# BaratiLab/LNS-Latent-Neural-PDE-Solver

Hardware: AMD Instinct MI355X
Metric: rollout-steps/sec (encode+N latent steps+decode), NS2d 128^2 3-ch (higher is better)
Workload: dtype f32 (f16x2 split operands on the fp16 MFMA pipe, fp32 accumulate; fp32 tensors in HBM); 1 GPU; NS2d 128x128 3-channel, 64-step latent rollout, batch=64 per GPU (BASELINE.json configs[1]); preset=ns2d_128, batch_per_gpu=64, rollout_steps=64, global_batch=64, parallelism=trajectory-sharded x1, streams=propagator + 3 decode streams per GPU

## Files before the change

include/lns.h:

```cpp
#ifndef LNS_H_
#define LNS_H_

#include <stddef.h>
#include <stdint.h>

#ifdef __cplusplus
extern "C" {
#endif

#define LNS_ABI_VERSION 2
#define LNS_MAX_STAGES 8
#define LNS_MAX_KEY 160

#define LNS_OK 0
#define LNS_EINVAL (-1)
#define LNS_ENOKEY (-2)
#define LNS_ESTATE (-3)
#define LNS_ENOMEM (-4)
#define LNS_EHIP (-5)
#define LNS_ENONFINITE (-6)

#define LNS_AE_NONE 0
#define LNS_AE_SQUARE 1
#define LNS_AE_NONSQUARED 2
// ... 459 lines not shown
                          double* lam, int32_t* status, void* stream);
int lns_op_ensemble_transform(const float* z, const double* X, int B, int M, int64_t n, float* out, void* stream);

int lns_op_energy_spectrum(const float* yhat, const float* y , int B, int T, int C, int H, int W,
                           const lns_eval_spec* spec, float* out, void* stream);
int lns_op_energy_spectrum_basis(const float* yhat, const float* y , int B, int T, int C, int H, int W,
                                 const lns_eval_spec* spec, float* out, void* stream, int basis_y, int basis_x);

int lns_op_field_stats(const float* yhat, const float* y, int B, int T, int C, int H, int W, const lns_eval_spec* spec,
                       const lns_stats_spec* hspec , float* stats_out, int32_t* hist_out ,
                       void* stream);

int lns_op_flow_stats(const float* yhat, const float* y, int B, int T, int C, int H, int W, const lns_eval_spec* spec,
                      const lns_flow_spec* fspec, float* flow_out, int32_t* hist_out , void* stream);
int lns_op_vorticity(const float* fields, int B, int T, int C, int H, int W, const lns_eval_spec* spec,
                     const lns_flow_spec* fspec, float* vort_out, void* stream);

int lns_time_maps_state_bytes(int B, int C, int H, int W, size_t* bytes);
int lns_op_time_maps(const float* yhat, const float* y, int B, int T, int C, int H, int W, const lns_eval_spec* spec,
                     int map_from, int map_every, float* maps_out, void* state, size_t state_bytes, void* stream);

int lns_op_eval_attrib(const float* yhat, const float* r, const float* y, int B, int T, int C, int H, int W,
                       const lns_eval_spec* spec, float* prop_frame, float* prop_seq, float* cross_frame, float* cross_seq,
                       void* stream);

int lns_op_latent_err(const float* z, const float* ztrue, int B, int T, int zper, int64_t zstride, float eps, float* frame_out,
                      float* seq_out, void* stream);

int lns_op_groupnorm_stats(const float* x, int B, int C, int HW, int groups, float eps,
                           const float* gamma_host, const float* beta_host, const float* premul,
                           float* ss, void* stream);
int lns_op_attention(const float* qkv, int B, int heads, int dim_head, int n, float scale,
                     float* o, void* stream);
int lns_op_fa_sandwich(const float* u, const float* kx, const float* ky, int B, int heads, int C,
                       int H, int W, float eps, int apply_instance_norm, float* out, void* stream);
int lns_op_fa_pool(const float* x, int64_t x_bs, const float* ss, int B, int C, int H, int W,
                   float* mx, float* my, void* stream);

int lns_op_fourier_block(const float* x, int B, int Cin, int Cout, int H, int W, int m1, int m2, const float* w1_host,
                         const float* w2_host, const float* conv_w_host, const float* conv_b_host,
                         const float* cond, const float* freq_w_host, const float* freq_b_host,
                         const float* lin_w_host, const float* lin_b_host, int activation, int residual,
                         float* y, void* stream);

typedef struct lns_fourier_block lns_fourier_block;
int lns_fourier_block_create(int Cin, int Cout, int m1, int m2, const float* w1_host, const float* w2_host,
                             const float* conv_w_host, const float* conv_b_host, const float* freq_w_host,
                             const float* freq_b_host, const float* lin_w_host, const float* lin_b_host, int activation,
                             int residual, int device, lns_fourier_block** out);
int lns_fourier_block_forward(lns_fourier_block* h, const float* x, const float* cond, int B, int H, int W, float* y,
                              void* stream);
void lns_fourier_block_destroy(lns_fourier_block* h);

int lns_metric_rel_l2(const float* yhat, const float* y, int B, int T, int C, int HW, float mean, float std, float eps,
                      float* frame_out, float* seq_out, float* scratch, void* stream);

#define LNS_METRIC_ZERO_WALLS 1
#define LNS_METRIC_CLAMP 2
int lns_metric_rel_l2_ch(const float* yhat, const float* y, int B, int T, int C, int H, int W, const float* mean_host,
                         const float* std_host, const int* flags_host, float clamp_lo, float clamp_hi, float eps,
                         float* frame_out, float* seq_out, float* scratch, void* stream);

#ifdef __cplusplus
}
#endif
#endif
// ... 1 lines not shown
```

lns-latent-neural-pde-solver_amd/_lib.py:

```python
import ctypes
import os
import subprocess

_HERE = os.path.dirname(os.path.abspath(__file__))
LIB_PATH = os.environ.get("LNS_HIP_LIB") or os.path.join(_HERE, "liblns_hip.so")
CSRC = os.path.join(_HERE, "csrc")

LNS_MAX_STAGES = 8
LNS_ABI_VERSION = 2
LNS_AE_NONE, LNS_AE_SQUARE, LNS_AE_NONSQUARED, LNS_AE_HALF_PERIODIC = 0, 1, 2, 3
LNS_PROP_NONE, LNS_PROP_PLAIN, LNS_PROP_CONDITIONAL = 0, 1, 2
LNS_PAD_ZEROS, LNS_PAD_CIRCULAR = 0, 1
LNS_SPECTRUM_DFT, LNS_SPECTRUM_DCT = 0, 1
LNS_OK, LNS_EINVAL, LNS_ENOKEY, LNS_ESTATE, LNS_ENOMEM, LNS_EHIP, LNS_ENONFINITE = 0, -1, -2, -3, -4, -5, -6


class LnsLibraryError(RuntimeError):
    pass


class LnsError(RuntimeError):
    pass


# ... 159 lines not shown


SYMBOLS = [
    "lns_create_error", "lns_create", "lns_destroy", "lns_last_error", "lns_num_params",
    "lns_param_info", "lns_set_weight", "lns_finalize_weights", "lns_latent_shape", "lns_prepare",
    "lns_encode", "lns_encode_cond", "lns_encode_affine", "lns_decode", "lns_propagate", "lns_rollout", "lns_rollout_latent", "lns_check_finite", "lns_set_option",
    "lns_rollout_eval_workspace_bytes", "lns_rollout_eval", "lns_rollout_latent_eval",
    "lns_rollout_select_workspace_bytes", "lns_rollout_select", "lns_rollout_latent_select",
    "lns_rollout_ensemble_workspace_bytes", "lns_rollout_latent_ensemble", "lns_op_ensemble_stats",
    "lns_rollout_latent_ensemble_eval", "lns_op_ensemble_score",
    "lns_rollout_latent_ensemble_quantiles", "lns_op_ensemble_quantiles",
    "lns_rollout_latent_ensemble_exceed", "lns_op_ensemble_exceed",
    "lns_rollout_ensemble_analysis_workspace_bytes", "lns_rollout_latent_ensemble_analysis",
    "lns_op_ensemble_obs_gram", "lns_op_etkf_transform", "lns_op_ensemble_transform",
    "lns_spectrum_bins", "lns_rollout_eval_spectrum", "lns_rollout_latent_eval_spectrum", "lns_op_energy_spectrum",
    "lns_spectrum_bins_basis", "lns_op_energy_spectrum_basis",
    "lns_rollout_eval_stats", "lns_rollout_latent_eval_stats", "lns_op_field_stats",
    "lns_rollout_eval_maps_workspace_bytes", "lns_rollout_eval_maps", "lns_rollout_latent_eval_maps",
    "lns_time_maps_state_bytes", "lns_op_time_maps",
    "lns_rollout_eval_attrib_workspace_bytes", "lns_rollout_eval_attrib", "lns_rollout_latent_eval_attrib",
    "lns_autoencode_eval_workspace_bytes", "lns_autoencode_eval", "lns_op_eval_attrib", "lns_op_latent_err",
    "lns_rollout_eval_flow", "lns_rollout_latent_eval_flow", "lns_op_flow_stats", "lns_op_vorticity",
    "lns_train_workspace_bytes", "lns_train_forward", "lns_train_backward",
    "lns_loss_smooth_l1", "lns_adam_step", "lns_adam_step_tensors", "lns_train_step_workspace_bytes", "lns_train_step",
    "lns_grad_norm_scratch_bytes", "lns_grad_norm_tensors", "lns_grad_scale_tensors", "lns_update_step_tensors",
    "lns_train_step_clip_workspace_bytes", "lns_train_step_clip",
    "lns_train_backward_ex", "lns_loss_obs_mse_scratch_bytes", "lns_loss_obs_mse", "lns_fit_step_workspace_bytes", "lns_fit_step",
    "lns_train_tangent_workspace_bytes", "lns_train_tangent", "lns_op_orthonormalize",
    "lns_trace_enable", "lns_trace_count", "lns_trace_info", "lns_trace_copy",
    "lns_timing_enable", "lns_timing_count", "lns_timing_info", "lns_timing_mfma_flops", "lns_build_has",
    "lns_op_conv_wgrad_scratch_bytes", "lns_op_conv_wgrad",
    "lns_op_groupnorm_train", "lns_op_gelu_grad", "lns_op_bias_grad",
    "lns_op_fa_reducer", "lns_fa_reducer_fits", "lns_op_fa_lrk", "lns_fa_lrk_fits", "lns_rotary_table", "lns_op_ln_pe", "lns_op_apply",
    "lns_op_conv2d", "lns_op_conv_gn", "lns_op_fa_fused", "lns_op_conv_pair_stress", "lns_op_groupnorm_stats", "lns_op_attention", "lns_op_fa_sandwich", "lns_op_fa_pool", "lns_op_fourier_block",
    "lns_fourier_block_create", "lns_fourier_block_forward", "lns_fourier_block_destroy", "lns_metric_rel_l2", "lns_metric_rel_l2_ch",
]

_lib = None


def build(force=False):
    srcs = [os.path.join(CSRC, f) for f in os.listdir(CSRC)
            if f.endswith((".hip", ".cpp", ".h", ".inc"))] + [os.path.join(_HERE, "..", "include", "lns.h")]
    if (not force and os.path.exists(LIB_PATH)
            and all(os.path.getmtime(LIB_PATH) >= os.path.getmtime(s) for s in srcs)):
        return LIB_PATH
    subprocess.check_call(["make", "-s", "-j4", "-C", CSRC])
    return LIB_PATH


def lib():
    global _lib
    if _lib is not None:
        return _lib
    if not os.path.exists(LIB_PATH):
        raise LnsLibraryError(
            "HIP extension %s is missing; run `python -c 'import __graft_entry__ as g; g.build()'` "
            "(there is no CPU fallback for the LNS hot path)" % LIB_PATH)
    try:
        L = ctypes.CDLL(LIB_PATH)
    except OSError as e:
        raise LnsLibraryError("cannot load %s: %s" % (LIB_PATH, e))
    c = ctypes
    vp, i, i64p, fp = c.c_void_p, c.c_int, c.POINTER(c.c_int64), c.POINTER(c.c_float)
    if os.environ.get("LNS_HIP_LIB"):
        def _absent(*_a, **_k):
            raise LnsLibraryError("entry point missing from the library selected by LNS_HIP_LIB")
# ... 133 lines not shown
    L.lns_build_has.argtypes = [c.c_char_p]
    L.lns_trace_enable.argtypes = [vp, i]
    L.lns_trace_count.argtypes = [vp]
    L.lns_trace_info.argtypes = [vp, i, c.c_char_p, i, i64p]
    L.lns_trace_copy.argtypes = [vp, i, vp]
    L.lns_timing_enable.argtypes = [vp, i]
    L.lns_timing_count.argtypes = [vp]
    L.lns_timing_info.argtypes = [vp, i, c.c_char_p, i, c.POINTER(c.c_double), i64p,
                                  c.POINTER(c.c_double), c.POINTER(c.c_double)]
    L.lns_timing_mfma_flops.argtypes = [vp, i, c.POINTER(c.c_double)]
    L.lns_op_conv2d.argtypes = [vp, i, i, i, i, i, i, vp, vp, i, i, i, i, i, i, i, i, i, i,
                                vp, i, i, vp, vp, vp, i, vp, vp]
    if hasattr(L, "lns_op_conv_gn"):
        L.lns_op_conv_gn.argtypes = [c.POINTER(LnsConvGnArgs), vp]
    if hasattr(L, "lns_op_fa_fused"):
        L.lns_op_fa_fused.argtypes = [c.POINTER(LnsFaFusedArgs), vp]
    if hasattr(L, "lns_op_fa_reducer"):
        L.lns_op_fa_reducer.argtypes = [c.POINTER(LnsFaReducerArgs), vp]
        L.lns_fa_reducer_fits.argtypes = [i, i, i, i]
        L.lns_op_fa_lrk.argtypes = [c.POINTER(LnsFaLrkArgs), vp]
        L.lns_fa_lrk_fits.argtypes = [i, i]
        L.lns_rotary_table.argtypes = [i, vp, i, vp]
        L.lns_op_ln_pe.argtypes = [vp, c.c_int64, i, i, i, vp, vp, vp, i, c.c_float, vp, fp, vp]
        L.lns_op_apply.argtypes = [vp, c.c_int64, vp, i, i, i, i, vp, vp, vp]
    if hasattr(L, "lns_op_conv_wgrad"):
        L.lns_op_conv_wgrad_scratch_bytes.argtypes = [i, i, i, i, i, i, i, c.POINTER(c.c_size_t)]
        L.lns_op_conv_wgrad.argtypes = [vp, vp, i, i, i, i, i, i, i, i, i, i, i, vp, vp, c.c_size_t, vp]
    if hasattr(L, "lns_op_groupnorm_train"):
        L.lns_op_groupnorm_train.argtypes = [vp, i, i, i, i, c.c_float, vp, vp, vp, vp, vp, vp, vp, vp, vp, i, vp, vp]
        L.lns_op_gelu_grad.argtypes = [vp, vp, vp, c.c_int64, vp]
        L.lns_op_bias_grad.argtypes = [vp, i, i, i, vp, i, vp]
    L.lns_op_groupnorm_stats.argtypes = [vp, i, i, i, i, c.c_float, vp, vp, vp, vp, vp]
    L.lns_op_attention.argtypes = [vp, i, i, i, i, c.c_float, vp, vp]
    L.lns_op_fa_sandwich.argtypes = [vp, vp, vp, i, i, i, i, i, c.c_float, i, vp, vp]
    L.lns_op_fa_pool.argtypes = [vp, c.c_int64, vp, i, i, i, i, vp, vp, vp]
    L.lns_op_fourier_block.argtypes = [vp, i, i, i, i, i, i, i, vp, vp, vp, vp, vp, vp, vp, vp, vp, i, i, vp, vp]
    L.lns_fourier_block_create.argtypes = [i, i, i, i, vp, vp, vp, vp, vp, vp, vp, vp, i, i, i, c.POINTER(vp)]
    L.lns_fourier_block_forward.argtypes = [vp, vp, vp, i, i, i, vp, vp]
    L.lns_fourier_block_destroy.argtypes = [vp]
    L.lns_fourier_block_destroy.restype = None
    L.lns_metric_rel_l2.argtypes = [vp, vp, i, i, i, i, c.c_float, c.c_float, c.c_float, vp, vp, vp, vp]
    L.lns_metric_rel_l2.restype = i
    L.lns_metric_rel_l2_ch.argtypes = [vp, vp, i, i, i, i, i, vp, vp, vp, c.c_float, c.c_float, c.c_float, vp, vp, vp, vp]
    L.lns_metric_rel_l2_ch.restype = i
    _lib = L
    return L
```

lns-latent-neural-pde-solver_amd/csrc/lns_engine.cpp:

```cpp
#include <algorithm>
#include <cmath>
#include <cstdarg>
#include <cstdio>
#include <cstdlib>
#include <cstring>
#include <memory>
#include <mutex>
#include <tuple>
#include <stdexcept>

#include "lns_conv_launch.h"
#include "lns_engine.h"
#include "lns_fold.h"
#include "lns_op_scratch.h"
#include "lns_resolve.h"
#include "lns_spectrum.h"

#define LNS_MAX_BATCH 65535

namespace lns {
void build_model(lns_engine* e);

static thread_local std::string g_create_error;

// ... 480 lines not shown
        TRef out = conv_same3(h1, l.conv2, 1, l.mode_y, l.mode_x, ACT_NONE, &skip, 0, l.name + ".conv2", raw_out);
        free_t(h1);
        if (skip_owned) free_t(skip);
        return out;
    }

    TRef lower_sa(const Layer& l, TRef x, bool raw_out) {
        if (x.pending()) throw std::runtime_error("SABlock input must be materialised");
        const int n = x.H * x.W, inner = l.heads * l.dim_head;
        if (l.pe >= 0 && n > l.pe_len) throw std::runtime_error("SABlock: more tokens than positional table rows");
        TRef h = alloc_t(x.C, x.H, x.W);
        h.amax_const = ln_pe_bound(x.C, vec_absmax(l.ln_g), vec_absmax(l.ln_b), vec_absmax(l.pe));
        {
            Op op;
            op.type = OP_LNPE; op.name = l.name + ".ln_pe"; op.cls = CLS_LNPE;
            memset(&op.ln, 0, sizeof op.ln);
            op.ln.x = as_ptr<const float>(x.ptr); op.ln.x_bs = x.bs; op.ln.C = x.C; op.ln.n = n; op.ln.eps = 1e-5f;
            op.ln.gamma = as_ptr<const float>(vecp(l.ln_g)); op.ln.beta = as_ptr<const float>(vecp(l.ln_b));
            op.ln.pe_t = as_ptr<const float>(vecp(l.pe)); op.ln.pe_stride = l.pe_len;
            op.ln.h = as_ptr<float>(h.ptr); op.ln.B = B;
            op.bytes = 2.0 * B * x.C * n * 4;
            plan->ops.push_back(op);
        }
        TRef qkv = conv_same1(h, l.qkv, ACT_NONE, nullptr, nullptr, l.name + ".qkv");
        free_t(h);
        TRef o = alloc_t(inner, x.H, x.W);
        o.amax = qkv.amax;
        {
            Op op;
            op.type = OP_ATTN; op.name = l.name + ".attn"; op.cls = CLS_ATTN;
            op.at.qkv = as_ptr<const float>(qkv.ptr); op.at.B = B; op.at.heads = l.heads; op.at.D = l.dim_head;
            op.at.n = n; op.at.scale = (float)std::pow((double)l.dim_head, -0.5); op.at.o = as_ptr<float>(o.ptr);
            op.at.amax_in = qkv.amax ? as_ptr<const unsigned>(qkv.amax) : nullptr;
            op.flops = 4.0 * B * l.heads * (double)n * n * l.dim_head;
            {
                const bool f16 = op.at.amax_in != nullptr && getenv("LNS_ATTN_FP32") == nullptr;
                const double np_ = (n + 31) / 32 * 32;
                op.mfma_flops = 4.0 * B * l.heads * np_ * np_ * l.dim_head * (f16 ? 3.0 : 1.0);
                op.form = f16 ? "f16x2 attention" : "fp32 MFMA attention";
            }
            op.bytes = 4.0 * B * 4.0 * inner * n;
            plan->ops.push_back(op);
        }
        free_t(qkv);
        TRef out = conv_same1(o, l.proj, ACT_NONE, &x, nullptr, l.name + ".proj_out", -1, raw_out);
        free_t(o);
        return out;
    }

    uint64_t rotary_table(int n, const std::string& invf_key) {
        const Param& p = e->params[e->pindex.at(invf_key)];
        const int half = (int)p.numel();
        std::vector<float> cs((size_t)n * half * 2);
        rotary_table_fill(n, p.host.data(), half, cs.data());
        return const_floats(cs);
    }

    int next_chunk_group = 1;
    int fa_chunk_samples(size_t bytes_per_sample) const {
        const long cap = (long)e->opt_fa_chunk_mb << 20;
        if (cap <= 0 || (long)bytes_per_sample * B <= cap) return 0;
        const int chunk = (int)std::max<long>(1, cap / (long)bytes_per_sample);
        return chunk >= B ? 0 : chunk;
    }
    void chunk_fa_chain(size_t inproj_at, size_t sandwich_at, size_t toout_at, size_t bytes_per_sample) {
        const int chunk = fa_chunk_samples(bytes_per_sample);
// ... 1036 lines not shown

using namespace lns;

struct DeviceGuard {
    int prev = -1; bool switched = false;
    explicit DeviceGuard(const lns_engine* e) : DeviceGuard(e->device) {}
    explicit DeviceGuard(int device) {
        if (device >= 0 && hipGetDevice(&prev) == hipSuccess && prev != device)
            switched = hipSetDevice(device) == hipSuccess;
    }
    ~DeviceGuard() { if (switched) (void)hipSetDevice(prev); }
};



extern "C" {

const char* lns_create_error(void) { return g_create_error.c_str(); }

int lns_create(const lns_config* cfg, lns_engine** out) {
    if (!cfg || !out) { g_create_error = "null argument"; return LNS_EINVAL; }
    if (cfg->abi_version != LNS_ABI_VERSION) { g_create_error = "ABI version mismatch"; return LNS_EINVAL; }
    lns_engine* e = new lns_engine();
    e->cfg = *cfg;
    if (const char* v = getenv("LNS_DECODE_GROUP")) e->opt_decode_group = atoi(v);
    if (const char* v = getenv("LNS_DECODE_STREAMS")) e->opt_decode_streams = atoi(v);
    if (getenv("LNS_NO_OVERLAP")) e->opt_overlap = 0;
    if (getenv("LNS_PROP_PRIORITY")) e->opt_prop_priority = 1;
    if (const char* v = getenv("LNS_FA_CHUNK_MB")) e->opt_fa_chunk_mb = atoi(v);
    if (const char* v = getenv("LNS_FA_FUSED")) e->opt_fa_fused = std::min(3, std::max(0, atoi(v)));
    if (const char* v = getenv("LNS_FA_FUSED_GPB")) e->opt_fa_fused_gpb = std::max(0, atoi(v));
    if (getenv("LNS_NO_FOLD_LINEAR")) e->opt_fold_linear = 0;
    if (const char* v = getenv("LNS_UP2_DUAL")) e->opt_up2_dual = atoi(v) != 0;
    e->cfg.ae_prefix[sizeof(e->cfg.ae_prefix) - 1] = 0;
    e->cfg.prop_prefix[sizeof(e->cfg.prop_prefix) - 1] = 0;
    try {
        build_model(e);
    } catch (const std::exception& ex) {
        g_create_error = ex.what();
        delete e;
        return LNS_EINVAL;
    }
    *out = e;
    return LNS_OK;
}

void lns_train_release(const lns_engine* e);

void lns_destroy(lns_engine* e) {
    if (!e) return;
    lns_train_release(e);
    drop_plans(e, true);
    if (e->d_weights) (void)hipFree(e->d_weights);
    if (e->d_sticky) (void)hipFree(e->d_sticky);
    release_overlap_objects(e);
    delete e;
}

const char* lns_last_error(const lns_engine* e) { return e ? e->err.c_str() : "null engine"; }

int lns_num_params(const lns_engine* e) { return e ? (int)e->params.size() : LNS_EINVAL; }

int lns_param_info(const lns_engine* e, int index, char* key, int key_capacity, int64_t* shape, int* ndim,
                   int* is_buffer) {
    if (!e || index < 0 || index >= (int)e->params.size()) return LNS_EINVAL;
    const Param& p = e->params[index];
// ... 22 lines not shown

int lns_finalize_weights(lns_engine* e, int device) {
    if (!e) return LNS_EINVAL;
    return finalize_weights(e, device);
}

int lns_set_option(lns_engine* e, const char* name, long value) {
    if (!e || !name) return LNS_EINVAL;
    const std::string n = name;
    auto set_rule = [e, value](int& opt) { if (opt != (int)value) { DeviceGuard dg(e); drop_plans(e, false); } opt = (int)value; };
    if (n == "decode_group") { if (value < 0 || value > 8) return LNS_EINVAL; e->opt_decode_group = (int)value; }
    else if (n == "decode_streams") { if (value < 1 || value > NDEC) return LNS_EINVAL; e->opt_decode_streams = (int)value; }
    else if (n == "overlap") e->opt_overlap = value != 0;
    else if (n == "eval_max_steps") { if (value < 1 || value > 65536) return LNS_EINVAL; e->opt_eval_max_steps = (int)value; }
    else if (n == "track_nonfinite") e->opt_track_nonfinite = value != 0;
    else if (n == "train_wgrad") {
        if (value != 0 && value != 1) { e->err = "train_wgrad: 0 (one block per output tile) or 1 (batch-parallel)"; return LNS_EINVAL; }
        e->opt_train_wgrad = (int)value;
    }
    else if (n == "spectrum_basis") {
        if (value < 0 || value > 3) { e->err = "spectrum_basis: basis_y | basis_x << 1 with LNS_SPECTRUM_DFT (0) or LNS_SPECTRUM_DCT (1), i.e. 0 .. 3"; return LNS_EINVAL; }
        e->opt_spectrum_basis = (int)value;
        return LNS_OK;
    }
    else if (n == "fa_fused") { if (value < 0 || value > 3) return LNS_EINVAL; set_rule(e->opt_fa_fused); }
    else if (n == "fa_fused_gpb") { if (value < 0 || value > 64) return LNS_EINVAL; set_rule(e->opt_fa_fused_gpb); }
    else if (n == "fold_linear") {
        if (value != 0 && value != 1) { e->err = "fold_linear: 0 (the pair as it stands) or 1 (one conv on the composed weights)"; return LNS_EINVAL; }
        set_rule(e->opt_fold_linear);
    }
    else if (n == "up2_dual") {
        if (value != 0 && value != 1) { e->err = "up2_dual: 0 (one block per output phase) or 1 (both column phases per block where the form fits)"; return LNS_EINVAL; }
        set_rule(e->opt_up2_dual);
    }
    else if (n == "fa_chunk_mb") { if (value < 0 || value > 4096) return LNS_EINVAL; set_rule(e->opt_fa_chunk_mb); }
    else if (n == "prop_priority") {
        if (e->opt_prop_priority != (value != 0)) { DeviceGuard dg(e); release_overlap_objects(e); }
        e->opt_prop_priority = value != 0;
    } else { e->err = "unknown option: " + n; return LNS_EINVAL; }
    e->ran.clear(); e->ran_ws = nullptr; e->ran_B = 0;
    return LNS_OK;
}

int lns_latent_shape(const lns_engine* e, int* C, int* H, int* W) {
    if (!e || e->enc.empty()) return LNS_EINVAL;
    if (C) *C = e->lat_C;
    if (H) *H = e->lat_H;
    if (W) *W = e->lat_W;
    return LNS_OK;
}

static int check_batch(lns_engine* e, int B) {
    if (B > LNS_MAX_BATCH) { e->err = fmt("batch %d exceeds the maximum of %d trajectories per call", B, LNS_MAX_BATCH); return LNS_EINVAL; }
    return LNS_OK;
}

static int einval(lns_engine* e, const char* what) { e->err = what; return LNS_EINVAL; }

static int need_model(lns_engine* e) {
    if (e->enc.empty() || e->prop.empty()) { e->err = "rollout needs autoencoder and propagator"; return LNS_ESTATE; }
    return LNS_OK;
}

static int need_param(lns_engine* e, bool encodes, const float* param) {
    if (param) return LNS_OK;
    if (e->cfg.prop_kind == LNS_PROP_CONDITIONAL || (encodes && e->cfg.cond_encoder))
// ... 1220 lines not shown
```

lns-latent-neural-pde-solver_amd/csrc/lns_engine.h:

```cpp
#pragma once
#include <map>
#include <string>
#include <vector>

#include "../../include/lns.h"
#include "lns_kernels.h"

namespace lns {

struct Param {
    std::string key;
    std::vector<int64_t> shape;
    std::vector<float> host;
    bool is_buffer = false;
    bool is_set = false;
    size_t numel() const { size_t n = 1; for (auto s : shape) n *= (size_t)s; return n; }
};

struct ConvPack {
    std::vector<std::string> wkeys;
    std::vector<std::string> bkeys;
    std::vector<int> couts;
    int cin = 0, cout = 0, k = 1;
    bool has_bias = false;
// ... 88 lines not shown

struct TraceRec { std::string name; int B, C, H, W; std::vector<float> data; };
struct TimeRec { std::string name; double ms = 0; int64_t launches = 0; double flops = 0, bytes = 0, mfma_flops = 0; };

}

struct lns_engine {
    lns_config cfg;
    std::string err;
    std::vector<lns::Param> params;
    std::map<std::string, int> pindex;
    std::vector<lns::ConvPack> packs;
    std::vector<lns::VecPack> vecs;
    std::vector<lns::Layer> enc, dec, prop;
    int lat_C = 0, lat_H = 0, lat_W = 0;
    float* d_weights = nullptr;
    size_t weights_floats = 0;
    bool finalized = false;
    int device = -1;
    std::map<long, lns::Plan> enc_plans, dec_plans, prop_plans;
    void* side_stream = nullptr;
    std::vector<hipStream_t> dec_streams;
    std::vector<hipEvent_t> events;
    int opt_decode_group = 1;
    int opt_decode_streams = 3;
    int opt_eval_max_steps = 1024;
    int opt_overlap = 1;
    int opt_prop_priority = 0;
    int opt_fa_chunk_mb = 0;
    int opt_fa_fused = 2;
    int opt_fa_fused_gpb = 0;
    int opt_fold_linear = 1;
    int opt_up2_dual = 1;
    struct RanRec { int kind; long key; size_t arena_off; };
    std::vector<RanRec> ran;
    const void* ran_ws = nullptr;
    int ran_B = 0;
    int opt_track_nonfinite = 0;
    int opt_spectrum_basis = 0;
    int opt_train_wgrad = 0;
    unsigned* d_sticky = nullptr;
    bool sticky_armed = false;
    bool trace_on = false;
    std::vector<lns::TraceRec> trace;
    bool timing_on = false;
    std::vector<lns::TimeRec> timing;
    double timing_overhead_ms = -1.0;
};
```

lns-latent-neural-pde-solver_amd/csrc/lns_kernels.h:

```cpp
#pragma once
#include <hip/hip_runtime.h>
#include <stdint.h>

namespace lns {

enum Act { ACT_NONE = 0, ACT_SWISH = 1, ACT_GELU = 2, ACT_RELU = 3, ACT_TANH = 4, ACT_SIGMOID = 5 };

template <class A, class F> void for_each_stride(A&, F&&) {}
#define LNS_ARGS_SIZE(T, n) static_assert(sizeof(T) == (n), "member added to " #T ": list it in for_each_ptr if it is a pointer, in for_each_stride if it is a tagged batch stride")

struct ConvArgs {
    const float* x;
    long x_bs;
    int Cin, Hin, Win;
    const float* w;
    const float* bias;
    const float* ss;
    int act_in, act_out;
    const int* rowmap;
    const int* colmap;
    float* y;
    long y_bs;
    int y_bdiv; long y_bs2;
    int Cout, Hout, Wout;
// ... 88 lines not shown
hipError_t launch_conv1_bf16x3(const ConvArgs& a, hipStream_t s);
bool conv1_thin_fits(const ConvArgs& a);
hipError_t launch_conv1_thin(const ConvArgs& a, hipStream_t s);

struct GnStatsArgs {
    const float* x; long x_bs; int C, HW, groups; float eps;
    const float* gamma; const float* beta;
    const float* premul;
    float* ss;
    int B;
};
template <class F> void for_each_ptr(GnStatsArgs& a, F&& f) { f(a.x); f(a.gamma); f(a.beta); f(a.premul); f(a.ss); }
template <class F> void for_each_stride(GnStatsArgs& a, F&& f) { f(a.x_bs); }
LNS_ARGS_SIZE(GnStatsArgs, 72);
bool gn_stats_two_stage(const GnStatsArgs& a);
hipError_t launch_gn_stats(const GnStatsArgs& a, float* part, hipStream_t s);
#define GN_TILE_PIXELS 128
struct GnTileGeom { int tiles_x, bw_log2, H, W, flat; };
hipError_t launch_gn_tile_finalize(const GnStatsArgs& a, const float* tile_part, int tiles, int count, GnTileGeom geom, hipStream_t s);

struct LnPeArgs {
    const float* x; long x_bs; int C, n; float eps;
    const float* gamma; const float* beta;
    const float* pe_t;
    int pe_stride;
    float* h;
    int B;
};
template <class F> void for_each_ptr(LnPeArgs& a, F&& f) { f(a.x); f(a.gamma); f(a.beta); f(a.pe_t); f(a.h); }
template <class F> void for_each_stride(LnPeArgs& a, F&& f) { f(a.x_bs); }
LNS_ARGS_SIZE(LnPeArgs, 80);
hipError_t launch_ln_pe(const LnPeArgs& a, hipStream_t s);

struct AttnArgs { const float* qkv; int B, heads, D, n; float scale; float* o;
                  const unsigned* amax_in; };
template <class F> void for_each_ptr(AttnArgs& a, F&& f) { f(a.qkv); f(a.o); f(a.amax_in); }
LNS_ARGS_SIZE(AttnArgs, 48);
hipError_t launch_attention(const AttnArgs& a, hipStream_t s);

struct FaPoolArgs { const float* x; long x_bs; const float* ss; int B, C, H, W; float* mx; float* my; };
template <class F> void for_each_ptr(FaPoolArgs& a, F&& f) { f(a.x); f(a.ss); f(a.mx); f(a.my); }
template <class F> void for_each_stride(FaPoolArgs& a, F&& f) { f(a.x_bs); }
LNS_ARGS_SIZE(FaPoolArgs, 56);
hipError_t launch_fa_pool(const FaPoolArgs& a, hipStream_t s);

struct FaReducerArgs {
    const float* m; long rows; int n;
    int C, Hid, Out;
    const float* win_t;
    const float* ln_g; const float* ln_b;
    const float* w1_t;
    const float* w2_t;
    const float* b2;
    float* u;
    unsigned* amax_out;
    const float* wqk_t; int ldqk;
    const float* bqk;
    int Mqk; float* qk;
};
template <class F> void for_each_ptr(FaReducerArgs& a, F&& f) {
    f(a.m); f(a.win_t); f(a.ln_g); f(a.ln_b); f(a.w1_t); f(a.w2_t); f(a.b2); f(a.u); f(a.amax_out); f(a.wqk_t); f(a.bqk); f(a.qk);
}
LNS_ARGS_SIZE(FaReducerArgs, 136);
hipError_t launch_fa_reducer(const FaReducerArgs& a, hipStream_t s);
hipError_t launch_fa_reducer2(const FaReducerArgs& ax, const FaReducerArgs& ay, hipStream_t s);

struct FaLrkArgs {
    const float* qk;
// ... 249 lines not shown
```

lns-latent-neural-pde-solver_amd/csrc/lns_kernels.hip:

```cpp
#include <cstdlib>
#include <type_traits>

#include "lns_kernels.h"
#include "lns_spectrum.h"

namespace lns {

#ifndef LNS_CONV_STORE_AUX
#define LNS_CONV_STORE_AUX 0
#endif
#ifndef LNS_NTS_CONV3F
#define LNS_NTS_CONV3F 0
#endif
#ifndef LNS_NTS_CONV1F
#define LNS_NTS_CONV1F 0
#endif
#ifndef LNS_SAND_STORE_AUX
#define LNS_SAND_STORE_AUX 0
#endif
typedef float f32x16 __attribute__((ext_vector_type(16)));

__device__ __forceinline__ float gelu_erfc(float v) {
    const float z = fabsf(v) * 0.70710678118654752440f;
    const float t = __builtin_amdgcn_rcpf(fmaf(0.5f, z, 1.0f));
// ... 2979 lines not shown
        uint4 ph[2], pl[2];
#pragma unroll
        for (int tp = 0; tp < 2; ++tp) {
            unsigned hq[4], lq[4];
#pragma unroll
            for (int e = 0; e < 4; ++e) split2_pair_f16(sacc[8 * tp + 2 * e] * SP, sacc[8 * tp + 2 * e + 1] * SP, hq[e], lq[e]);
            ph[tp] = make_uint4(hq[0], hq[1], hq[2], hq[3]);
            pl[tp] = make_uint4(lq[0], lq[1], lq[2], lq[3]);
        }
#pragma unroll
        for (int mt = 0; mt < D / 32; ++mt) {
#pragma unroll
            for (int r = 0; r < 16; ++r) oacc[mt][r] *= alpha;
#pragma unroll
            for (int tp = 0; tp < 2; ++tp) {
                const f16x8 vh_ = *reinterpret_cast<const f16x8*>(va + (0 * D + mt * 32) * (VW * 2) + tp * 32);
                const f16x8 vl_ = *reinterpret_cast<const f16x8*>(va + (1 * D + mt * 32) * (VW * 2) + tp * 32);
                oacc[mt] = __builtin_amdgcn_mfma_f32_32x32x16_f16(vh_, __builtin_bit_cast(f16x8, ph[tp]), oacc[mt], 0, 0, 0);
                oacc[mt] = __builtin_amdgcn_mfma_f32_32x32x16_f16(vh_, __builtin_bit_cast(f16x8, pl[tp]), oacc[mt], 0, 0, 0);
                oacc[mt] = __builtin_amdgcn_mfma_f32_32x32x16_f16(vl_, __builtin_bit_cast(f16x8, ph[tp]), oacc[mt], 0, 0, 0);
            }
        }
    }
    if (qvalid) {
        const float inv = (SPINV * sinv) / l;
        float* ob = a.o + ((long)b * inner + (long)h * D) * n + query;
#pragma unroll
        for (int mt = 0; mt < D / 32; ++mt)
#pragma unroll
            for (int r = 0; r < 16; ++r) ob[(long)(mt * 32 + drow(r, kh)) * n] = oacc[mt][r] * inv;
    }
}

hipError_t launch_attention(const AttnArgs& a, hipStream_t s) {
    dim3 grid((a.n + 127) / 128, a.heads, a.B);
    static const bool fp32_only = getenv("LNS_ATTN_FP32") != nullptr;
    if (a.amax_in && !fp32_only) {
        if (a.D == 64) hipLaunchKernelGGL(attention_f_kernel<64>, grid, dim3(256), 0, s, a);
        else if (a.D == 32) hipLaunchKernelGGL(attention_f_kernel<32>, grid, dim3(256), 0, s, a);
        else return hipErrorInvalidValue;
        return hipGetLastError();
    }
    if (a.D == 64) hipLaunchKernelGGL(attention_kernel<64>, grid, dim3(256), 0, s, a);
    else if (a.D == 32) hipLaunchKernelGGL(attention_kernel<32>, grid, dim3(256), 0, s, a);
    else return hipErrorInvalidValue;
    return hipGetLastError();
}

__global__ __launch_bounds__(256) void fa_pool_kernel(FaPoolArgs a) {
    extern __shared__ __attribute__((aligned(16))) char smem[];
    float* P = reinterpret_cast<float*>(smem);
    const int c = blockIdx.x, b = blockIdx.y;
    const int H = a.H, W = a.W, WP = W + 1;
    const float* vs = a.x + (long)b * a.x_bs + (long)c * H * W;
    float sc = 1.0f, sh = 0.0f;
    if (a.ss) { const float2 st = *reinterpret_cast<const float2*>(a.ss + ((long)b * a.C + c) * 2); sc = st.x; sh = st.y; }
    for (int i = threadIdx.x; i < H * W; i += 256) {
        const int y = i / W, x = i - y * W;
        P[y * WP + x] = vs[i];
    }
    __syncthreads();
    for (int y = threadIdx.x; y < H; y += 256) {
        float s = 0.0f;
        for (int x = 0; x < W; ++x) s += P[y * WP + x];
        a.mx[((long)b * H + y) * a.C + c] = fmaf(s / (float)W, sc, sh);
    }
    for (int x = threadIdx.x; x < W; x += 256) {
        float s = 0.0f;
        for (int y = 0; y < H; ++y) s += P[y * WP + x];
// ... 1779 lines not shown
        constexpr bool UL = HT * WT >= 6;                                                                                \
        LNS_SET_LDS((fa_sandwich_b_kernel<HT, WT, true, (HT == WT), NWV, UL>))                                           \
        LNS_SET_LDS((fa_sandwich_b_kernel<HT, WT, true, false, NWV, UL>))                                                \
        LNS_SET_LDS((fa_sandwich_b_kernel<HT, WT, false, false, NWV, UL>))                                               \
    }
    LNS_SET_SWB(1, 1) LNS_SET_SWB(1, 2) LNS_SET_SWB(2, 1) LNS_SET_SWB(2, 2) LNS_SET_SWB(2, 3)
#undef LNS_SET_SWB
#define LNS_SET_SWF(HT, WT)                                                                                              \
    {                                                                                                                    \
        constexpr bool ULF = false;                                                                                      \
        LNS_SET_LDS((fa_sandwich_f_kernel<HT, WT, true, (HT == WT), ULF>))                                               \
        LNS_SET_LDS((fa_sandwich_f_kernel<HT, WT, true, false, ULF>))                                                    \
        LNS_SET_LDS((fa_sandwich_f_kernel<HT, WT, false, false, ULF>))                                                   \
    }
    LNS_SET_SWF(1, 1) LNS_SET_SWF(1, 2) LNS_SET_SWF(2, 1) LNS_SET_SWF(2, 2) LNS_SET_SWF(2, 3)
#undef LNS_SET_SWF
    LNS_SET_LDS((fa_fused_kernel<2>))
    LNS_SET_LDS((fa_fused2_kernel<2>))
    LNS_SET_LDS((fa_fused_g_kernel<2, 2, 2>))
    LNS_SET_LDS((fa_fused_g_kernel<4, 1, 1>))
    LNS_SET_LDS((fa_fused_g_kernel<2, 1, 1>))
    LNS_SET_LDS((fa_sandwich_kernel<1, 1, true>))
    LNS_SET_LDS((fa_sandwich_kernel<1, 1, false>))
    LNS_SET_LDS((fa_sandwich_kernel<1, 2, true>))
    LNS_SET_LDS((fa_sandwich_kernel<1, 2, false>))
    LNS_SET_LDS((fa_sandwich_kernel<2, 2, true>))
    LNS_SET_LDS((fa_sandwich_kernel<2, 2, false>))
    LNS_SET_LDS((fa_sandwich_kernel<2, 3, true>))
    LNS_SET_LDS((fa_sandwich_kernel<2, 3, false>))
    LNS_SET_LDS((fa_sandwich_kernel<2, 1, true>))
    LNS_SET_LDS((fa_sandwich_kernel<2, 1, false>))
    LNS_SET_LDS((conv1s_bf16x3_kernel<true>))
    LNS_SET_LDS((conv1s_bf16x3_kernel<false>))
    LNS_SET_LDS((conv1_bf16x3_kernel<true, true>))
    LNS_SET_LDS((conv1_bf16x3_kernel<true, false>))
    LNS_SET_LDS((conv1_bf16x3_kernel<false, true>))
    LNS_SET_LDS((conv1_bf16x3_kernel<false, false>))
    LNS_SET_LDS((conv3_bf16x3_kernel<1, 1, false, 2, 2>))
    LNS_SET_LDS((conv3_bf16x3_kernel<1, 1, false, 2, 2, 4>))
    LNS_SET_LDS((conv3_bf16x3_kernel<1, 2, false, 2, 2, 4>))
    LNS_SET_LDS((conv3_bf16x3_kernel<1, 1, true, 2, 2, 4>))
    LNS_SET_LDS((conv3_bf16x3_kernel<1, 2, true, 2, 2, 4>))
    LNS_SET_LDS((conv3_bf16x3_kernel<1, 1, false, 2, 2, 9, true>))
    LNS_SET_LDS((conv3_bf16x3_kernel<1, 2, false, 2, 2, 9, true>))
    LNS_SET_LDS((conv3_bf16x3_kernel<1, 1, true, 2, 2, 9, true>))
    LNS_SET_LDS((conv3_bf16x3_kernel<1, 2, true, 2, 2, 9, true>))
    LNS_SET_LDS((conv3_bf16x3_kernel<1, 1, false, 2, 2, 4, true>))
    LNS_SET_LDS((conv3_bf16x3_kernel<1, 2, false, 2, 2, 4, true>))
    LNS_SET_LDS((conv3_bf16x3_kernel<1, 1, true, 2, 2, 4, true>))
    LNS_SET_LDS((conv3_bf16x3_kernel<1, 2, true, 2, 2, 4, true>))
    LNS_SET_LDS((conv3_bf16x3_kernel<1, 1, false, 1, 2, 9, true>))
    LNS_SET_LDS((conv3_bf16x3_kernel<1, 2, false, 1, 2, 9, true>))
    LNS_SET_LDS((conv3_bf16x3_kernel<2, 2, false, 2, 2>))
    LNS_SET_LDS((conv3_bf16x3_kernel<2, 2, true, 2, 2>))
    LNS_SET_LDS((conv3_bf16x3_kernel<1, 2, false, 2, 2>))
    LNS_SET_LDS((conv3_bf16x3_kernel<1, 1, true, 2, 2>))
    LNS_SET_LDS((conv3_bf16x3_kernel<1, 2, true, 2, 2>))
    LNS_SET_LDS((conv3_bf16x3_kernel<1, 1, false, 1>))
    LNS_SET_LDS((conv3_bf16x3_kernel<1, 1, false, 1, 2>))
    LNS_SET_LDS((conv3_bf16x3_kernel<1, 2, false, 1, 2>))
    LNS_SET_LDS((conv3_bf16x3_kernel<1, 2, false, 1>))
    LNS_SET_LDS((conv3_bf16x3_kernel<1, 1, true>))
    LNS_SET_LDS((conv3_bf16x3_kernel<1, 1, false>))
    LNS_SET_LDS((conv3_bf16x3_kernel<1, 2, true>))
    LNS_SET_LDS((conv3_bf16x3_kernel<1, 2, false>))
    LNS_SET_LDS(fa_reducer_mfma_kernel)
// ... 16 lines not shown
```

lns-latent-neural-pde-solver_amd/csrc/lns_ops.inc:

```
#define OPCHK(call)                                                                                   \
    do { hipError_t err__ = (call);                                                                   \
         if (err__ != hipSuccess) { fprintf(stderr, "lns_op: %s: %s\n", #call, hipGetErrorString(err__)); return LNS_EHIP; } } while (0)

static int op_refuse(const char* op, const std::string& m) { g_create_error = std::string(op) + ": " + m; return LNS_EINVAL; }

struct OpConv {
    ConvArgs a;
    int variant = -1;
    OpScratch mem;
    float* dw = nullptr;
    int* dmaps = nullptr;
    unsigned* damax = nullptr;
    bool defer_amax = false;
    void release() { mem.release(); dw = nullptr; dmaps = nullptr; damax = nullptr; }
};

static int op_conv_prepare(OpConv& oc, const float* x, int B, int Cin, int Hin, int Win, int Hv, int Wv,
                           const float* w_host, const float* bias_host, int Cout, int ksize, int stride, int dilation,
                           int pad_t, int pad_b, int pad_l, int pad_r, int mode_y, int mode_x, const float* ss, int act_in,
                           int act_out, const float* residual, const float* badd, float* y, int tile_variant, hipStream_t stream) {
    if (!x || !w_host || !y || (ksize != 1 && ksize != 3)) return LNS_EINVAL;
    if (act_in != ACT_NONE && act_in != ACT_SWISH) return LNS_EINVAL;
    OPCHK(init_kernels());
    const int layout = tile_variant >= 0 ? (tile_variant & 0x300) : 0;
// ... 614 lines not shown
        (!frame_out && !seq_out))
        return LNS_EINVAL;
    MetricChannelSpec spec;
    for (int c = 0; c < LNS_METRIC_MAX_CH; ++c) {
        spec.mean[c] = (mean_host && c < C) ? mean_host[c] : 0.0f;
        spec.std[c] = (std_host && c < C) ? std_host[c] : 1.0f;
        spec.flags[c] = (flags_host && c < C) ? flags_host[c] : 0;
    }
    spec.lo = clamp_lo; spec.hi = clamp_hi;
    OPCHK(launch_metric_rel_l2_ch(yhat, y, B, T, C, H, W, spec, eps, frame_out, seq_out, scratch, static_cast<hipStream_t>(stream)));
    return LNS_OK;
}

int lns_op_groupnorm_stats(const float* x, int B, int C, int HW, int groups, float eps, const float* gamma_host,
                           const float* beta_host, const float* premul, float* ss, void* stream) {
    if (!x || !ss || C % groups) return LNS_EINVAL;
    OpScratch sc;
    float* dgb = static_cast<float*>(sc.alloc((size_t)2 * C));
    OPCHK(sc.err);
    if (gamma_host) sc.copy_in(dgb, gamma_host, C);
    if (beta_host) sc.copy_in(dgb + C, beta_host, C);
    GnStatsArgs a;
    memset(&a, 0, sizeof a);
    a.x = x; a.x_bs = (long)C * HW; a.C = C; a.HW = HW; a.groups = groups; a.eps = eps;
    a.gamma = gamma_host ? dgb : nullptr; a.beta = beta_host ? dgb + C : nullptr; a.premul = premul; a.ss = ss; a.B = B;
    hipStream_t s = static_cast<hipStream_t>(stream);
    float* part = static_cast<float*>(sc.alloc((size_t)B * C * 2));
    if (sc.ok()) sc.note(launch_gn_stats(a, part, s));
    OPCHK(sc.finish(s));
    return LNS_OK;
}

int lns_op_attention(const float* qkv, int B, int heads, int dim_head, int n, float scale, float* o, void* stream) {
    if (!qkv || !o) return LNS_EINVAL;
    AttnArgs a = {qkv, B, heads, dim_head, n, scale, o, nullptr};
    hipStream_t s = static_cast<hipStream_t>(stream);
    OpScratch sc;
    unsigned* damax = sc.amax_words(B, s);
    const long per = 3L * heads * dim_head * n;
    if (sc.ok()) sc.note(launch_amax(qkv, per, per, B, damax, s));
    a.amax_in = damax;
    if (sc.ok()) sc.note(launch_attention(a, s));
    OPCHK(sc.finish(s));
    return LNS_OK;
}

int lns_op_fa_sandwich(const float* u, const float* kx, const float* ky, int B, int heads, int C, int H, int W, float eps,
                       int apply_instance_norm, float* out, void* stream) {
    if (!u || !kx || !ky || !out) return LNS_EINVAL;
    OPCHK(init_kernels());
    FaSandwichArgs a = {u, kx, ky, B, heads, C, H, W, eps, apply_instance_norm, out, nullptr, 0};
    hipStream_t s = static_cast<hipStream_t>(stream);
    OpScratch sc;
    unsigned* damax = sc.amax_words(B, s);
    if (sc.ok()) sc.note(launch_amax(u, (long)heads * C * H * W, (long)heads * C * H * W, B, damax, s));
    a.amax_u = damax;
    if (sc.ok()) sc.note(launch_fa_sandwich(a, s));
    OPCHK(sc.finish(s));
    return LNS_OK;
}

int lns_op_fa_pool(const float* x, int64_t x_bs, const float* ss, int B, int C, int H, int W, float* mx, float* my, void* stream) {
    if (!x || !mx || !my || B <= 0 || C <= 0 || H <= 0 || W <= 0 || x_bs < (int64_t)C * H * W) return LNS_EINVAL;
    OPCHK(init_kernels());
    FaPoolArgs a = {x, (long)x_bs, ss, B, C, H, W, mx, my};
    hipStream_t s = static_cast<hipStream_t>(stream);
    OPCHK(launch_fa_pool(a, s));
    OPCHK(hipStreamSynchronize(s));
// ... 330 lines not shown
```

Baseline: 40970 trajectory-steps/s.

## Add wide attention kernel with 256-query blocks and double-buffered K/V in LDS

Adds a 512-thread attention kernel in which each block handles 256 queries per sample and head. K/V tiles of 64 keys are staged as f16 hi/lo splits in double-buffered LDS, with global prefetch overlapped with the MFMA steps. The kernel is used by default when a per-sample amax exists, D is 32 or 64, and n > 128. The aim is to raise K/V reuse per load and cut redundant global reads compared with the 128-query kernel. The cost is larger LDS use and higher register pressure, which may reduce occupancy.

After: 41050 trajectory-steps/s (median of 2 runs). About the same (+0.2%).

```diff
diff --git a/include/lns.h b/include/lns.h
--- a/include/lns.h
+++ b/include/lns.h
@@ -515,6 +515,8 @@
                            float* ss, void* stream);
 int lns_op_attention(const float* qkv, int B, int heads, int dim_head, int n, float scale,
                      float* o, void* stream);
+int lns_op_attention_form(const float* qkv, int B, int heads, int dim_head, int n, float scale,
+                          float* o, int form, void* stream);
 int lns_op_fa_sandwich(const float* u, const float* kx, const float* ky, int B, int heads, int C,
                        int H, int W, float eps, int apply_instance_norm, float* out, void* stream);
 int lns_op_fa_pool(const float* x, int64_t x_bs, const float* ss, int B, int C, int H, int W,
diff --git a/lns-latent-neural-pde-solver_amd/_lib.py b/lns-latent-neural-pde-solver_amd/_lib.py
--- a/lns-latent-neural-pde-solver_amd/_lib.py
+++ b/lns-latent-neural-pde-solver_amd/_lib.py
@@ -215,7 +215,7 @@
     "lns_op_conv_wgrad_scratch_bytes", "lns_op_conv_wgrad",
     "lns_op_groupnorm_train", "lns_op_gelu_grad", "lns_op_bias_grad",
     "lns_op_fa_reducer", "lns_fa_reducer_fits", "lns_op_fa_lrk", "lns_fa_lrk_fits", "lns_rotary_table", "lns_op_ln_pe", "lns_op_apply",
-    "lns_op_conv2d", "lns_op_conv_gn", "lns_op_fa_fused", "lns_op_conv_pair_stress", "lns_op_groupnorm_stats", "lns_op_attention", "lns_op_fa_sandwich", "lns_op_fa_pool", "lns_op_fourier_block",
+    "lns_op_conv2d", "lns_op_conv_gn", "lns_op_fa_fused", "lns_op_conv_pair_stress", "lns_op_groupnorm_stats", "lns_op_attention", "lns_op_attention_form", "lns_op_fa_sandwich", "lns_op_fa_pool", "lns_op_fourier_block",
     "lns_fourier_block_create", "lns_fourier_block_forward", "lns_fourier_block_destroy", "lns_metric_rel_l2", "lns_metric_rel_l2_ch",
 ]
 
@@ -415,6 +415,7 @@
         L.lns_op_bias_grad.argtypes = [vp, i, i, i, vp, i, vp]
     L.lns_op_groupnorm_stats.argtypes = [vp, i, i, i, i, c.c_float, vp, vp, vp, vp, vp]
     L.lns_op_attention.argtypes = [vp, i, i, i, i, c.c_float, vp, vp]
+    L.lns_op_attention_form.argtypes = [vp, i, i, i, i, c.c_float, vp, i, vp]
     L.lns_op_fa_sandwich.argtypes = [vp, vp, vp, i, i, i, i, i, c.c_float, i, vp, vp]
     L.lns_op_fa_pool.argtypes = [vp, c.c_int64, vp, i, i, i, i, vp, vp, vp]
     L.lns_op_fourier_block.argtypes = [vp, i, i, i, i, i, i, i, vp, vp, vp, vp, vp, vp, vp, vp, vp, i, i, vp, vp]
diff --git a/lns-latent-neural-pde-solver_amd/csrc/attention_w.inc b/lns-latent-neural-pde-solver_amd/csrc/attention_w.inc
--- /dev/null
+++ b/lns-latent-neural-pde-solver_amd/csrc/attention_w.inc
@@ -0,0 +1,197 @@
+#ifndef ATTN_W_WAVES
+#define ATTN_W_WAVES 4
+#endif
+constexpr int ATTN_W_QUERIES = 256, ATTN_W_KEYS = 64;
+__host__ __device__ constexpr int attn_w_lds_bytes(int D) { return 2 * (2 * ATTN_W_KEYS * (D + 8) + 2 * D * (ATTN_W_KEYS + 8)) * 2; }
+
+template <int D>
+__global__ __launch_bounds__(512, ATTN_W_WAVES) void attention_w_kernel(AttnArgs a) {
+    constexpr int KW = D + 8, VW = ATTN_W_KEYS + 8;
+    constexpr int KT = 2 * ATTN_W_KEYS * KW, VT = 2 * D * VW;
+    extern __shared__ __attribute__((aligned(16))) char smem[];
+    unsigned short* Kb = reinterpret_cast<unsigned short*>(smem);
+    unsigned short* Vb = Kb + 2 * KT;
+    const int tid = threadIdx.x, lane = tid & 63, wave = tid >> 6;
+    const int l31 = lane & 31, kh = lane >> 5;
+    const int h = blockIdx.y, b = blockIdx.z;
+    const int n = a.n;
+    const long inner = (long)a.heads * D;
+    const float* qb = a.qkv + ((long)b * 3 * inner + (long)h * D) * n;
+    const float* kb = qb + inner * n;
+    const float* vb = kb + inner * n;
+    const int query = (blockIdx.x * 8 + wave) * 32 + l31;
+    const bool qvalid = query < n;
+    const bool wave_on = (blockIdx.x * 8 + wave) * 32 < n;
+    float sinv;
+    const float sc = f16x2_scale(amax_load(a.amax_in, b), sinv);
+    constexpr float SP = 16384.0f, SPINV = 1.0f / 16384.0f;
+
+    uint4 qh[D / 16], ql[D / 16];
+    {
+        float qv[D / 16][8];
+        const unsigned qlane = qvalid ? (unsigned)(8 * kh * n + query) * 4u : 0u;
+#pragma unroll
+        for (int t = 0; t < D / 16; ++t)
+#pragma unroll
+            for (int e = 0; e < 8; ++e) {
+                const char* row = reinterpret_cast<const char*>(qb + (long)(16 * t + e) * n);
+                const float v = *reinterpret_cast<const float*>(row + qlane);
+                qv[t][e] = qvalid ? v : 0.0f;
+            }
+#pragma unroll
+        for (int t = 0; t < D / 16; ++t) {
+            unsigned hq[4], lq[4];
+#pragma unroll
+            for (int e = 0; e < 4; ++e) split2_pair_f16(qv[t][2 * e] * sc, qv[t][2 * e + 1] * sc, hq[e], lq[e]);
+            qh[t] = make_uint4(hq[0], hq[1], hq[2], hq[3]);
+            ql[t] = make_uint4(lq[0], lq[1], lq[2], lq[3]);
+        }
+    }
+    float m = -INFINITY, l = 0.0f;
+    f32x16 oacc[D / 32];
+#pragma unroll
+    for (int mt = 0; mt < D / 32; ++mt)
+#pragma unroll
+        for (int r = 0; r < 16; ++r) oacc[mt][r] = 0.0f;
+
+    const int ntile = (n + ATTN_W_KEYS - 1) / ATTN_W_KEYS;
+    constexpr bool ALL = D == 64;
+    const int kkey = tid & 63, koct = __builtin_amdgcn_readfirstlane(tid >> 6);
+    const int vd = tid >> 3, voct = tid & 7;
+    const bool kact = ALL || koct < D / 8, vact = ALL || vd < D;
+    float pre[8];
+    const float* krow = kb + (long)(kact ? 8 * koct : 0) * n;
+    const unsigned vlane = vact ? (unsigned)(vd * n) * 4u : 0u;
+    auto fetch_k = [&](int kt) __attribute__((always_inline)) {
+        const int key = kt * ATTN_W_KEYS + kkey;
+        const bool ok = kact && key < n;
+        const unsigned ko = ok ? (unsigned)key * 4u : 0u;
+#pragma unroll
+        for (int e = 0; e < 8; ++e) {
+            const float v = *reinterpret_cast<const float*>(reinterpret_cast<const char*>(krow + (long)e * n) + ko);
+            pre[e] = ok ? v : 0.0f;
+        }
+    };
+    auto fetch_v = [&](int kt) __attribute__((always_inline)) {
+        const int k0 = kt * ATTN_W_KEYS + 8 * voct;
+#pragma unroll
+        for (int e = 0; e < 8; ++e) {
+            const bool ok = vact && k0 + e < n;
+            const float v = *reinterpret_cast<const float*>(reinterpret_cast<const char*>(vb) + (ok ? vlane + (unsigned)(k0 + e) * 4u : 0u));
+            pre[e] = ok ? v : 0.0f;
+        }
+    };
+    auto stage_k = [&](int buf) __attribute__((always_inline)) {
+        unsigned short* Ks = Kb + buf * KT;
+        if (kact) {
+            unsigned hq[4], lq[4];
+#pragma unroll
+            for (int e = 0; e < 4; ++e) split2_pair_f16(pre[2 * e] * sc, pre[2 * e + 1] * sc, hq[e], lq[e]);
+            *reinterpret_cast<uint4*>(Ks + (0 * ATTN_W_KEYS + kkey) * KW + 8 * koct) = make_uint4(hq[0], hq[1], hq[2], hq[3]);
+            *reinterpret_cast<uint4*>(Ks + (1 * ATTN_W_KEYS + kkey) * KW + 8 * koct) = make_uint4(lq[0], lq[1], lq[2], lq[3]);
+        }
+    };
+    auto stage_v = [&](int buf) __attribute__((always_inline)) {
+        unsigned short* Vs = Vb + buf * VT;
+        if (vact) {
+            unsigned hq[4], lq[4];
+#pragma unroll
+            for (int e = 0; e < 4; ++e) split2_pair_f16(pre[2 * e] * sc, pre[2 * e + 1] * sc, hq[e], lq[e]);
+            const int blk = (voct >> 1) * 16, p0 = blk + (voct & 1) * 4, p1 = p0 + 8;
+            *reinterpret_cast<uint2*>(Vs + (0 * D + vd) * VW + p0) = make_uint2(hq[0], hq[1]);
+            *reinterpret_cast<uint2*>(Vs + (0 * D + vd) * VW + p1) = make_uint2(hq[2], hq[3]);
+            *reinterpret_cast<uint2*>(Vs + (1 * D + vd) * VW + p0) = make_uint2(lq[0], lq[1]);
+            *reinterpret_cast<uint2*>(Vs + (1 * D + vd) * VW + p1) = make_uint2(lq[2], lq[3]);
+        }
+    };
+    auto step = [&](const unsigned short* Ks, const unsigned short* Vs, int hs, int key0) __attribute__((always_inline)) {
+        const char* ka = reinterpret_cast<const char*>(Ks) + ((hs * 32 + l31) * KW + 8 * kh) * 2;
+        const char* va = reinterpret_cast<const char*>(Vs) + (l31 * VW + 8 * kh) * 2 + hs * 64;
+        f32x16 sacc;
+#pragma unroll
+        for (int r = 0; r < 16; ++r) sacc[r] = 0.0f;
+#pragma unroll
+        for (int t = 0; t < D / 16; ++t) {
+            if (t) __builtin_amdgcn_sched_barrier(0);
+            const f16x8 kh_ = *reinterpret_cast<const f16x8*>(ka + t * 32);
+            const f16x8 kl_ = *reinterpret_cast<const f16x8*>(ka + ATTN_W_KEYS * KW * 2 + t * 32);
+            sacc = __builtin_amdgcn_mfma_f32_32x32x16_f16(kh_, __builtin_bit_cast(f16x8, qh[t]), sacc, 0, 0, 0);
+            sacc = __builtin_amdgcn_mfma_f32_32x32x16_f16(kh_, __builtin_bit_cast(f16x8, ql[t]), sacc, 0, 0, 0);
+            sacc = __builtin_amdgcn_mfma_f32_32x32x16_f16(kl_, __builtin_bit_cast(f16x8, qh[t]), sacc, 0, 0, 0);
+        }
+        const float sscale = (a.scale * sinv) * sinv;
+        float tmax = -INFINITY;
+#pragma unroll
+        for (int r = 0; r < 16; ++r) {
+            const int key = key0 + drow(r, kh);
+            float sv = sacc[r] * sscale;
+            if (key >= n) sv = -INFINITY;
+            sacc[r] = sv;
+            tmax = fmaxf(tmax, sv);
+        }
+        tmax = fmaxf(tmax, __shfl_xor(tmax, 32));
+        const float mnew = fmaxf(m, tmax);
+        const float alpha = __builtin_amdgcn_exp2f((m - mnew) * 1.44269504088896341f);
+        float lt = 0.0f;
+#pragma unroll
+        for (int r = 0; r < 16; ++r) {
+            const float p = __builtin_amdgcn_exp2f((sacc[r] - mnew) * 1.44269504088896341f);
+            sacc[r] = p;
+            lt += p;
+        }
+        lt += __shfl_xor(lt, 32);
+        l = l * alpha + lt;
+        m = mnew;
+#pragma unroll
+        for (int mt = 0; mt < D / 32; ++mt)
+#pragma unroll
+            for (int r = 0; r < 16; ++r) oacc[mt][r] *= alpha;
+#pragma unroll
+        for (int tp = 0; tp < 2; ++tp) {
+            __builtin_amdgcn_sched_barrier(0);
+            unsigned hq[4], lq[4];
+#pragma unroll
+            for (int e = 0; e < 4; ++e) split2_pair_f16(sacc[8 * tp + 2 * e] * SP, sacc[8 * tp + 2 * e + 1] * SP, hq[e], lq[e]);
+            const f16x8 ph = __builtin_bit_cast(f16x8, make_uint4(hq[0], hq[1], hq[2], hq[3]));
+            const f16x8 pl = __builtin_bit_cast(f16x8, make_uint4(lq[0], lq[1], lq[2], lq[3]));
+#pragma unroll
+            for (int mt = 0; mt < D / 32; ++mt) {
+                const f16x8 vh_ = *reinterpret_cast<const f16x8*>(va + (0 * D + mt * 32) * (VW * 2) + tp * 32);
+                const f16x8 vl_ = *reinterpret_cast<const f16x8*>(va + (1 * D + mt * 32) * (VW * 2) + tp * 32);
+                oacc[mt] = __builtin_amdgcn_mfma_f32_32x32x16_f16(vh_, ph, oacc[mt], 0, 0, 0);
+                oacc[mt] = __builtin_amdgcn_mfma_f32_32x32x16_f16(vh_, pl, oacc[mt], 0, 0, 0);
+                oacc[mt] = __builtin_amdgcn_mfma_f32_32x32x16_f16(vl_, ph, oacc[mt], 0, 0, 0);
+            }
+        }
+        __builtin_amdgcn_sched_barrier(0);
+    };
+
+    fetch_k(0);
+    stage_k(0);
+    fetch_v(0);
+    stage_v(0);
+    __syncthreads();
+    for (int kt = 0; kt < ntile; ++kt) {
+        const int key0 = kt * ATTN_W_KEYS, buf = kt & 1;
+        const bool next = kt + 1 < ntile;
+        const unsigned short* Ks = Kb + buf * KT;
+        const unsigned short* Vs = Vb + buf * VT;
+        if (next) fetch_k(kt + 1);
+        if (wave_on) step(Ks, Vs, 0, key0);
+        if (next) { stage_k(buf ^ 1); fetch_v(kt + 1); }
+        if (wave_on && key0 + 32 < n) step(Ks, Vs, 1, key0 + 32);
+        if (next) stage_v(buf ^ 1);
+        __syncthreads();
+    }
+    int tid2 = threadIdx.x;
+    asm volatile("" : "+v"(tid2));
+    const int query2 = (blockIdx.x * 8 + (tid2 >> 6)) * 32 + (tid2 & 31);
+    if (query2 < n) {
+        const float inv = (SPINV * sinv) / l;
+        float* ob = a.o + ((long)b * inner + (long)h * D) * n + query2;
+#pragma unroll
+        for (int mt = 0; mt < D / 32; ++mt)
+#pragma unroll
+            for (int r = 0; r < 16; ++r) ob[(long)(mt * 32 + drow(r, kh)) * n] = oacc[mt][r] * inv;
+    }
+}
diff --git a/lns-latent-neural-pde-solver_amd/csrc/lns_engine.cpp b/lns-latent-neural-pde-solver_amd/csrc/lns_engine.cpp
--- a/lns-latent-neural-pde-solver_amd/csrc/lns_engine.cpp
+++ b/lns-latent-neural-pde-solver_amd/csrc/lns_engine.cpp
@@ -536,6 +536,7 @@
             op.at.qkv = as_ptr<const float>(qkv.ptr); op.at.B = B; op.at.heads = l.heads; op.at.D = l.dim_head;
             op.at.n = n; op.at.scale = (float)std::pow((double)l.dim_head, -0.5); op.at.o = as_ptr<float>(o.ptr);
             op.at.amax_in = qkv.amax ? as_ptr<const unsigned>(qkv.amax) : nullptr;
+            op.at.wide = e->opt_sa_forms;
             op.flops = 4.0 * B * l.heads * (double)n * n * l.dim_head;
             {
                 const bool f16 = op.at.amax_in != nullptr && getenv("LNS_ATTN_FP32") == nullptr;
@@ -1638,6 +1639,7 @@
     if (const char* v = getenv("LNS_FA_FUSED_GPB")) e->opt_fa_fused_gpb = std::max(0, atoi(v));
     if (getenv("LNS_NO_FOLD_LINEAR")) e->opt_fold_linear = 0;
     if (const char* v = getenv("LNS_UP2_DUAL")) e->opt_up2_dual = atoi(v) != 0;
+    if (const char* v = getenv("LNS_SA_FORMS")) e->opt_sa_forms = atoi(v) != 0;
     e->cfg.ae_prefix[sizeof(e->cfg.ae_prefix) - 1] = 0;
     e->cfg.prop_prefix[sizeof(e->cfg.prop_prefix) - 1] = 0;
     try {
@@ -1726,6 +1728,10 @@
     else if (n == "up2_dual") {
         if (value != 0 && value != 1) { e->err = "up2_dual: 0 (one block per output phase) or 1 (both column phases per block where the form fits)"; return LNS_EINVAL; }
         set_rule(e->opt_up2_dual);
+    }
+    else if (n == "sa_forms") {
+        if (value != 0 && value != 1) { e->err = "sa_forms: 0 (attention in blocks of 128 queries) or 1 (one attention block per sample, head and 256 queries where the form applies)"; return LNS_EINVAL; }
+        set_rule(e->opt_sa_forms);
     }
     else if (n == "fa_chunk_mb") { if (value < 0 || value > 4096) return LNS_EINVAL; set_rule(e->opt_fa_chunk_mb); }
     else if (n == "prop_priority") {
diff --git a/lns-latent-neural-pde-solver_amd/csrc/lns_engine.h b/lns-latent-neural-pde-solver_amd/csrc/lns_engine.h
--- a/lns-latent-neural-pde-solver_amd/csrc/lns_engine.h
+++ b/lns-latent-neural-pde-solver_amd/csrc/lns_engine.h
@@ -144,6 +144,7 @@
     int opt_fa_fused_gpb = 0;
     int opt_fold_linear = 1;
     int opt_up2_dual = 1;
+    int opt_sa_forms = 1;
     struct RanRec { int kind; long key; size_t arena_off; };
     std::vector<RanRec> ran;
     const void* ran_ws = nullptr;
diff --git a/lns-latent-neural-pde-solver_amd/csrc/lns_kernels.h b/lns-latent-neural-pde-solver_amd/csrc/lns_kernels.h
--- a/lns-latent-neural-pde-solver_amd/csrc/lns_kernels.h
+++ b/lns-latent-neural-pde-solver_amd/csrc/lns_kernels.h
@@ -144,8 +144,11 @@
 LNS_ARGS_SIZE(LnPeArgs, 80);
 hipError_t launch_ln_pe(const LnPeArgs& a, hipStream_t s);
 
-struct AttnArgs { const float* qkv; int B, heads, D, n; float scale; float* o;
+struct AttnArgs { const float* qkv; int B, heads, D, n; float scale;
+                  int wide;
+                  float* o;
                   const unsigned* amax_in; };
+bool attn_wide_fits(int D, int n, bool has_amax);
 template <class F> void for_each_ptr(AttnArgs& a, F&& f) { f(a.qkv); f(a.o); f(a.amax_in); }
 LNS_ARGS_SIZE(AttnArgs, 48);
 hipError_t launch_attention(const AttnArgs& a, hipStream_t s);
diff --git a/lns-latent-neural-pde-solver_amd/csrc/lns_kernels.hip b/lns-latent-neural-pde-solver_amd/csrc/lns_kernels.hip
--- a/lns-latent-neural-pde-solver_amd/csrc/lns_kernels.hip
+++ b/lns-latent-neural-pde-solver_amd/csrc/lns_kernels.hip
@@ -3035,9 +3035,20 @@
     }
 }
 
+#include "attention_w.inc"
+
+bool attn_wide_fits(int D, int n, bool has_amax) { return has_amax && (D == 64 || D == 32) && n > 128; }
+
 hipError_t launch_attention(const AttnArgs& a, hipStream_t s) {
+    if (a.D != 64 && a.D != 32) return hipErrorInvalidValue;
     dim3 grid((a.n + 127) / 128, a.heads, a.B);
     static const bool fp32_only = getenv("LNS_ATTN_FP32") != nullptr;
+    if (a.wide && !fp32_only && attn_wide_fits(a.D, a.n, a.amax_in != nullptr)) {
+        dim3 gw((a.n + ATTN_W_QUERIES - 1) / ATTN_W_QUERIES, a.heads, a.B);
+        if (a.D == 64) hipLaunchKernelGGL(attention_w_kernel<64>, gw, dim3(512), attn_w_lds_bytes(64), s, a);
+        else hipLaunchKernelGGL(attention_w_kernel<32>, gw, dim3(512), attn_w_lds_bytes(32), s, a);
+        return hipGetLastError();
+    }
     if (a.amax_in && !fp32_only) {
         if (a.D == 64) hipLaunchKernelGGL(attention_f_kernel<64>, grid, dim3(256), 0, s, a);
         else if (a.D == 32) hipLaunchKernelGGL(attention_f_kernel<32>, grid, dim3(256), 0, s, a);
@@ -4883,6 +4894,8 @@
     LNS_SET_LDS((fa_sandwich_kernel<2, 1, false>))
     LNS_SET_LDS((conv1s_bf16x3_kernel<true>))
     LNS_SET_LDS((conv1s_bf16x3_kernel<false>))
+    LNS_SET_LDS(attention_w_kernel<64>)
+    LNS_SET_LDS(attention_w_kernel<32>)
     LNS_SET_LDS((conv1_bf16x3_kernel<true, true>))
     LNS_SET_LDS((conv1_bf16x3_kernel<true, false>))
     LNS_SET_LDS((conv1_bf16x3_kernel<false, true>))
diff --git a/lns-latent-neural-pde-solver_amd/csrc/lns_ops.inc b/lns-latent-neural-pde-solver_amd/csrc/lns_ops.inc
--- a/lns-latent-neural-pde-solver_amd/csrc/lns_ops.inc
+++ b/lns-latent-neural-pde-solver_amd/csrc/lns_ops.inc
@@ -670,8 +670,14 @@
 }
 
 int lns_op_attention(const float* qkv, int B, int heads, int dim_head, int n, float scale, float* o, void* stream) {
-    if (!qkv || !o) return LNS_EINVAL;
-    AttnArgs a = {qkv, B, heads, dim_head, n, scale, o, nullptr};
+    return lns_op_attention_form(qkv, B, heads, dim_head, n, scale, o, -1, stream);
+}
+
+int lns_op_attention_form(const float* qkv, int B, int heads, int dim_head, int n, float scale, float* o, int form, void* stream) {
+    if (!qkv || !o || form < -1 || form > 1) return LNS_EINVAL;
+    if (form == 1 && !attn_wide_fits(dim_head, n, true)) return LNS_EINVAL;
+    OPCHK(init_kernels());
+    AttnArgs a = {qkv, B, heads, dim_head, n, scale, form != 0 ? 1 : 0, o, nullptr};
     hipStream_t s = static_cast<hipStream_t>(stream);
     OpScratch sc;
     unsigned* damax = sc.amax_words(B, s);
```
